# zetareticula/diffusion-llm-rs

Hardware: AMD Instinct MI355X
Metric: int4 dequant+GEMM GiB/s & tok/s per denoise step, 4096×4096, 1/2/4/8 GPU (higher is better)
Workload: dtype f16 X x exact int4 weights (f32 group scales), f32 accumulate; 1 GPU; int4-g128 dequant+GEMM, M=4096 tokens x K=4096 x N=4096; M=4096, K=4096, N=4096, bits=4, group=128, parallelism=column-parallel (hidden dim) x1

## Files before the change

diffusion-llm-rs_amd/csrc/lab/attn_v4.inc:

```

template <int LAB = 0>
__global__ void __launch_bounds__(kWaves * 64)
kv_attention_kernel(const _Float16 *__restrict__ Q, const uint8_t *__restrict__ img, const float *__restrict__ kp,
                    const float *__restrict__ vp, int S, int H, _Float16 *__restrict__ O) {
    const int nkb = (S + kKB - 1) / kKB;
    __shared__ __attribute__((aligned(16))) AttnSmem sm;
    const int tid = threadIdx.x, lane = tid & 63, wave = tid >> 6;
    const int h = blockIdx.y;
    const int q0 = blockIdx.x * kQT + wave * 32;
    const int ql = lane & 31, hh = lane >> 5;
    const float ks = kp[0], vs = vp[0];
    const float c = 1.4426950408889634f * ks / sqrtf(static_cast<float>(kD));

    half8_t qf[kD / 16];
    {
        const int qrow = min(q0 + ql, S - 1);
        const _Float16 *qp = Q + (static_cast<size_t>(qrow) * H + h) * kD + 8 * hh;
#pragma unroll
        for (int t = 0; t < kD / 16; ++t) qf[t] = *reinterpret_cast<const half8_t *>(qp + 16 * t);
    }

    float16_t o[kD / 32];
#pragma unroll
    for (int dt = 0; dt < kD / 32; ++dt)
#pragma unroll
        for (int e = 0; e < 16; ++e) o[dt][e] = 0.0f;
    float m_run = -INFINITY, l_run = 0.0f;

    auto qk = [&](float16_t (&st)[2], const _Float16 (&kb_)[kKB][kKRow]) {
#pragma unroll
        for (int u = 0; u < 2; ++u) {
#pragma unroll
            for (int e = 0; e < 16; ++e) st[u][e] = 0.0f;
#pragma unroll
            for (int t = 0; t < kD / 16; ++t) {
                const half8_t kf = *reinterpret_cast<const half8_t *>(&kb_[32 * u + ql][16 * t + 8 * hh]);
                st[u] = __builtin_amdgcn_mfma_f32_32x32x16_f16(kf, qf[t], st[u], 0, 0, 0);
            }
        }
    };

    const uint8_t *himg = img + static_cast<size_t>(h) * nkb * kImg + lane * 16;
    const uint32_t wv = __builtin_amdgcn_readfirstlane(wave);
    constexpr bool STAG = false;
    auto dma_k = [&](int blk, int buf, uint32_t p0 = 0xffffffffu, uint32_t step = kWaves) {
        const uint8_t *src = himg + static_cast<size_t>(blk) * kImg;
        const uint32_t dst = __builtin_amdgcn_readfirstlane(lds_addr(&sm.k[buf][0][0]));
        for (uint32_t p = p0 == 0xffffffffu ? wv : p0; p < kKImg / 1024; p += step) glds16_asm(src + p * 1024, dst + p * 1024);
    };
    auto dma_v = [&](int blk, int buf, uint32_t p0 = 0xffffffffu, uint32_t step = kWaves) {
        const uint8_t *src = himg + static_cast<size_t>(blk) * kImg + kKImg;
        const uint32_t dst = __builtin_amdgcn_readfirstlane(lds_addr(&sm.vt[buf][0][0]));
        for (uint32_t p = p0 == 0xffffffffu ? wv : p0; p < kVImg / 1024; p += step) glds16_asm(src + p * 1024, dst + p * 1024);
    };
    const bool grp_b = STAG && wave >= kWaves / 2;
    auto raw_barrier = []() __attribute__((always_inline)) {
        asm volatile("s_waitcnt lgkmcnt(0)" ::: "memory");
        __builtin_amdgcn_s_barrier();
        __builtin_amdgcn_sched_barrier(0);
    };
    dma_k(0, 0);
    dma_v(0, 0);
    if (nkb > 1) dma_k(1, 1);
    if (STAG && nkb > 1) dma_v(1, 1);
    asm volatile("s_waitcnt vmcnt(0)" ::: "memory");
    __syncthreads();
    float16_t st[2], sn[2];
    qk(st, sm.k[0]);

    for (int kb = 0; kb < nkb; ++kb) {
        const int j0 = kb * kKB;
        const bool more1 = kb + 1 < nkb, more2 = kb + 2 < nkb;
        if (!(LAB & 2)) {
            if (more2) dma_k(kb + 2, kb & 1);
            if (more1) dma_v(kb + 1, (kb + 1) & 1);
        }
        if (more1) {
            if constexpr (LAB & 8) {
#pragma unroll
                for (int u = 0; u < 2; ++u) sn[u] = st[u] * 0.5f;
            } else {
                qk(sn, sm.k[(kb + 1) & 1]);
            }
        }

        if constexpr (LAB & 1) {
            float lsum = 0.0f;
#pragma unroll
            for (int u = 0; u < 2; ++u)
#pragma unroll
                for (int r = 0; r < 16; ++r) lsum += st[u][r];
            l_run += lsum;
        } else {
        float mloc = -INFINITY;
        if (__builtin_expect(j0 + kKB > S, 0)) {
            asm volatile("" ::: "memory");
#pragma unroll
            for (int u = 0; u < 2; ++u)
#pragma unroll
                for (int r = 0; r < 16; ++r) {
                    const int key = j0 + 32 * u + (r & 3) + 8 * (r >> 2) + 4 * hh;
                    st[u][r] = key < S ? st[u][r] : -INFINITY;
                }
        }
#pragma unroll
        for (int u = 0; u < 2; ++u)
#pragma unroll
            for (int r = 0; r < 16; ++r) mloc = fmaxf(mloc, st[u][r]);
        mloc = fmaxf(mloc, __shfl_xor(mloc, 32, 64));
        const float m_new = fmaxf(m_run, mloc * c);
        const float alpha = __builtin_amdgcn_exp2f(m_run - m_new);
        float lsum = 0.0f;
#pragma unroll
        for (int u = 0; u < 2; ++u)
#pragma unroll
            for (int r = 0; r < 16; ++r) {
                st[u][r] = __builtin_amdgcn_exp2f(fmaf(st[u][r], c, -m_new));
                lsum += st[u][r];
            }
        lsum += __shfl_xor(lsum, 32, 64);
        l_run = l_run * alpha + lsum;
        m_run = m_new;
        if (!__all(alpha == 1.0f)) {
            if (hh == 0) sm.bcast[wave][ql] = alpha;
            __builtin_amdgcn_s_waitcnt(0xC07F);
            __builtin_amdgcn_wave_barrier();
#pragma unroll
            for (int g = 0; g < 4; ++g) {
                const float4 a4 = *reinterpret_cast<const float4 *>(&sm.bcast[wave][8 * g + 4 * hh]);
#pragma unroll
                for (int dt = 0; dt < kD / 32; ++dt) {
                    o[dt][4 * g + 0] *= a4.x; o[dt][4 * g + 1] *= a4.y;
                    o[dt][4 * g + 2] *= a4.z; o[dt][4 * g + 3] *= a4.w;
                }
            }
        }
        }
        const auto &vt = sm.vt[kb & 1];
        if constexpr (!(LAB & 4)) {
// ... 45 lines not shown
```

diffusion-llm-rs_amd/csrc/lab/horner_lab_launch.inc:

```

namespace {

template <int MODE>
void launch_horner_t(const HornerGemmArgs &a, int y_f32, hipStream_t st, int grows = 0) {
    const int nbm = (a.M + 255) / 256, nbn = a.Npad / 256;
    const unsigned nb = static_cast<unsigned>(nbm * nbn);
    const PSampleEpi ep = a.epi ? *a.epi : PSampleEpi{};
    if (a.epi)
        wq_horner_kernel<float, 1, MODE><<<nb, 512, 0, st>>>(a.X, a.M, a.K, a.wdev, a.sz, a.hr, a.sf, a.bias,
                                                             a.epi->x_prev, a.N, a.Npad, nbm, nbn, ep, grows);
    else if (y_f32)
        wq_horner_kernel<float, 0, MODE><<<nb, 512, 0, st>>>(a.X, a.M, a.K, a.wdev, a.sz, a.hr, a.sf, a.bias,
                                                             static_cast<float *>(a.Y), a.N, a.Npad, nbm, nbn, ep,
                                                             grows);
    else
        wq_horner_kernel<__half, 0, MODE><<<nb, 512, 0, st>>>(a.X, a.M, a.K, a.wdev, a.sz, a.hr, a.sf, a.bias,
                                                              static_cast<__half *>(a.Y), a.N, a.Npad, nbm, nbn, ep,
                                                              grows);
}

int launch_horner_lab(const HornerGemmArgs &a, int y_f32, hipStream_t st) {
    if (a.lab == 44 || a.lab == 45) {
        if (a.lab == 44) launch_horner16_t<1 | 256 | 1024 | 2>(a, y_f32, st);
        else launch_horner16_t<1 | 256 | 1024 | 4096>(a, y_f32, st);
        DLLM_LAUNCH_CHECK();
        return DLLM_OK;
    }
    if (a.lab >= 40 && a.lab <= 43) {
        if (a.lab == 40) launch_horner16_t<1 | 256 | 1024 | 4>(a, y_f32, st);
        else if (a.lab == 41) launch_horner16_t<1 | 256 | 1024 | 4 | 8>(a, y_f32, st);
        else if (a.lab == 42) launch_horner16_t<1 | 256 | 1024 | 64>(a, y_f32, st);
        else launch_horner16_t<1 | 256 | 1024 | 2 | 4 | 8 | 64>(a, y_f32, st);
        DLLM_LAUNCH_CHECK();
        return DLLM_OK;
    }
    if (a.lab == 26 || a.lab == 27) {
        if (a.lab == 26) launch_horner16_t<256 | 1024>(a, y_f32, st);
        else launch_horner16_t<1 | 1024>(a, y_f32, st);
        DLLM_LAUNCH_CHECK();
        return DLLM_OK;
    }
    if (a.lab == 25) {
        launch_horner16_t<1 | 256 | 1024 | 2048>(a, y_f32, st);
        DLLM_LAUNCH_CHECK();
        return DLLM_OK;
    }
    if (a.lab == 24) {
        launch_horner16_t<1 | 256>(a, y_f32, st);
        DLLM_LAUNCH_CHECK();
        return DLLM_OK;
    }
    if (a.lab == 21) {
        launch_horner_t<1 | 256>(a, y_f32, st);
        DLLM_LAUNCH_CHECK();
        return DLLM_OK;
    }
    if (a.lab == 19 || a.lab == 20) {
        if (a.lab == 19) launch_horner_t<1 | 256 | 512>(a, y_f32, st);
        else launch_horner_t<3 | 4 | 8 | 16 | 64 | 512>(a, y_f32, st);
        return DLLM_OK;
    }
    if (a.lab == 17 || a.lab == 18) {
        if (a.lab == 17) launch_horner_t<3 | 4 | 8 | 16 | 32>(a, y_f32, st);
        else launch_horner_t<3 | 4 | 8 | 16 | 256>(a, y_f32, st);
        DLLM_LAUNCH_CHECK();
        return DLLM_OK;
    }
    if (a.lab == 16) {
        launch_horner_t<1>(a, y_f32, st);
        DLLM_LAUNCH_CHECK();
        return DLLM_OK;
    }
    if (a.lab == 14 || a.lab == 15) {
        if (a.lab == 14) launch_horner_t<3 | 4 | 8 | 16 | 64>(a, y_f32, st);
        else launch_horner_t<3 | 4 | 8 | 16 | 128>(a, y_f32, st);
        DLLM_LAUNCH_CHECK();
        return DLLM_OK;
    }
    if (a.lab >= 10 && a.lab <= 12) {
        launch_horner_t<1 | 256>(a, y_f32, st, a.lab == 10 ? 4 : a.lab == 11 ? 8 : 16);
        DLLM_LAUNCH_CHECK();
        return DLLM_OK;
    }
    if (a.lab >= 1 && a.lab <= 9) {
        if (a.lab == 1) launch_horner_t<0>(a, y_f32, st);
        else if (a.lab == 2) launch_horner_t<3>(a, y_f32, st);
        else if (a.lab == 3) launch_horner_t<2>(a, y_f32, st);
        else if (a.lab == 4) launch_horner_t<3 | 4>(a, y_f32, st);
        else if (a.lab == 5) launch_horner_t<3 | 8>(a, y_f32, st);
        else if (a.lab == 6) launch_horner_t<3 | 16>(a, y_f32, st);
        else if (a.lab == 7) launch_horner_t<3 | 4 | 8 | 16>(a, y_f32, st);
        else if (a.lab == 8) launch_horner_t<3 | 32>(a, y_f32, st);
        else launch_horner_t<3 | 64>(a, y_f32, st);
        DLLM_LAUNCH_CHECK();
        return DLLM_OK;
    }
    return fail(DLLM_ERR_INVALID_PARAMS, "unknown Horner lab variant");
}

}

int launch_horner_rows_gemm(const HornerGemmArgs &a, int rows, int y_f32, hipStream_t st) {
    if (rows != 128) return fail(DLLM_ERR_INVALID_PARAMS, "Horner tiles: 128 rows");
    launch_horner16_t<1 | 256, 8>(a, y_f32, st);
// ... 5 lines not shown
```

diffusion-llm-rs_amd/csrc/linear_horner.hip:

```cpp
#include "linear_common.hpp"

#include <type_traits>

#ifndef DLLM_LAB
#define DLLM_LAB 0
#endif

namespace dllm {
namespace {

constexpr int kHW = 8 * 1024;
constexpr int kHG = 2048;

__device__ __forceinline__ void horner_burst(__amdgpu_buffer_rsrc_t xr, uint32_t x0, uint32_t x1, uint32_t x2,
                                             uint32_t x3, uint32_t sx, __amdgpu_buffer_rsrc_t wr, uint32_t wo,
                                             uint32_t sw, uint32_t lds0) {
    uint32_t keep;
    asm volatile(
        "s_mov_b32 %0, m0\n\t"
        "s_mov_b32 m0, %9\n\t"
        "s_nop 0\n\t"
        "buffer_load_dwordx4 %1, %5, %6 offen lds\n\t"
        "s_add_u32 m0, m0, 0x2000\n\t"
        "s_nop 0\n\t"
// ... 300 lines not shown
            return;
        }
    }
    if (kg != 0) return;
    const bool vec_ok = (N % 4) == 0;
#pragma unroll
    for (int r = 0; r < 8; ++r) {
        const int m = m0 + r * 32 + (lane & 31);
        if (m >= M) continue;
        YT *yrow = Y + static_cast<size_t>(m) * N;
#pragma unroll
        for (int qd = 0; qd < 4; ++qd)
            store_out4<YT>(yrow, bias, nb0 + 8 * qd, N, vec_ok, acc[r][4 * qd + 0], acc[r][4 * qd + 1],
                           acc[r][4 * qd + 2], acc[r][4 * qd + 3]);
    }
}

typedef float fx4_t __attribute__((ext_vector_type(4)));
typedef uint32_t u32x4_t __attribute__((ext_vector_type(4)));

template <int TB>
__device__ __forceinline__ void store_tile16_f16_lds(uint8_t *img, const fx4_t (&acc)[TB][2], const float4 (&bv)[2],
                                                     __half *Y, int N, int m0, int n0, int wave, int lane) {
    constexpr int kRowB = 512, kCpr = 32;
    const int row16 = lane & 15, rq = lane >> 4;
    constexpr int kTPP = TB < 8 ? TB : 8;
#pragma unroll
    for (int p = 0; p < TB / kTPP; ++p) {
#pragma unroll
        for (int i = 0; i < kTPP; ++i) {
            const int t = 16 * i + row16;
#pragma unroll
            for (int cb = 0; cb < 2; ++cb) {
                const int pc = (4 * wave + 2 * cb + (rq >> 1)) ^ (t & (kCpr - 1));
                const fx4_t &a = acc[kTPP * p + i][cb];
                const float4 &b = bv[cb];
                union { __half h[4]; uint2 u; } pk;
                pk.h[0] = __float2half_rn(a[0] + b.x);
                pk.h[1] = __float2half_rn(a[1] + b.y);
                pk.h[2] = __float2half_rn(a[2] + b.z);
                pk.h[3] = __float2half_rn(a[3] + b.w);
                *reinterpret_cast<uint2 *>(img + t * kRowB + pc * 16 + (rq & 1) * 8) = pk.u;
            }
        }
        __syncthreads();
        const int c = lane % kCpr;
#pragma unroll
        for (int t0 = wave * 2; t0 < 16 * kTPP; t0 += 16) {
            const int t = t0 + lane / kCpr;
            const uint4 v = *reinterpret_cast<const uint4 *>(img + t * kRowB + ((c ^ (t & (kCpr - 1))) * 16));
#if DLLM_NT_STORE
            typedef unsigned int u4nt __attribute__((ext_vector_type(4)));
            __builtin_nontemporal_store(u4nt{v.x, v.y, v.z, v.w},
                                        reinterpret_cast<u4nt *>(Y + static_cast<size_t>(m0 + 16 * kTPP * p + t) * N + n0 + 8 * c));
#else
            *reinterpret_cast<uint4 *>(Y + static_cast<size_t>(m0 + 16 * kTPP * p + t) * N + n0 + 8 * c) = v;
#endif
        }
        __syncthreads();
    }
}

template <int TB>
struct H16 {
    static_assert(TB == 16 || TB == 8, "256- or 128-token tiles");
    static constexpr int kKPS = 16 / TB;
    static constexpr int kXB = 32 * 1024;
    static constexpr int kXSub = kXB / kKPS;
    static constexpr int kWB = kKPS * kHW;
    static constexpr int kStage = kXB + kWB + kHG;
    static constexpr int kNX = TB / 4;
    static constexpr int kPieces = kKPS * (kNX + 1) + 1;
};

template <typename YT, int EPI, int MODE, int TB = 16, int BITS = 4>
__global__ void __launch_bounds__(512, 1)
wq_horner16_kernel(const __half *__restrict__ X, int M, int K, const uint32_t *__restrict__ wdev,
                   const uint32_t *__restrict__ sz, const float *__restrict__ hr, const float *__restrict__ sf,
                   const float *__restrict__ bias, YT *__restrict__ Y, int N, int Npad, int nbm, int nbn,
                   PSampleEpi epi) {
    constexpr bool STAG = MODE & 1;
    static_assert(BITS == 4 || (BITS == 2 && TB == 16), "int4, or int2 on 256-token tiles");
    using L = H16<TB>;
    constexpr int kStage = L::kStage, kXB = L::kXB, kKPS = L::kKPS;
    __shared__ __attribute__((aligned(16))) uint8_t smem[3 * kStage];

    const int nb = nbm * nbn, orig = blockIdx.x;
    const int xcd = orig % kXCDs, q8 = nb / kXCDs, r8 = nb % kXCDs;
    const int tile = (xcd < r8 ? xcd * (q8 + 1) : r8 * (q8 + 1) + (xcd - r8) * q8) + orig / kXCDs;
    const int bm = tile / nbn, bn = tile % nbn;
    const int lane = threadIdx.x & 63;
    const int wave = __builtin_amdgcn_readfirstlane(threadIdx.x >> 6);
    const int m0 = bm * 16 * TB, n0 = bn * 256;
    const int nk = K / kBK;
    const int ns = nk / kKPS;

    uint32_t xo[L::kNX];
#pragma unroll
    for (int i = 0; i < L::kNX; ++i) {
        const int row = (i * 8 + wave) * 8 + (lane >> 3);
        const int rrow = (m0 + row < M ? m0 + row : M - 1) - m0;
        const int c = (lane & 7) ^ ((row >> 1) & 5);
        xo[i] = static_cast<uint32_t>((rrow * K + c * 8) * 2);
    }
    const __amdgpu_buffer_rsrc_t xr = raw_rsrc(X + static_cast<size_t>(m0) * K);
    const uint32_t nt = static_cast<uint32_t>(n0 + 32 * wave) >> 5;
    const __amdgpu_buffer_rsrc_t wr = raw_rsrc(wdev + static_cast<size_t>(nt) * nk * 64 * BITS);
    auto wsoff = [](int kstep) { return static_cast<uint32_t>(BITS == 4 ? kstep * 1024 : (kstep & ~1) * 512); };
    const uint32_t wo = static_cast<uint32_t>(lane * 16);
    const __amdgpu_buffer_rsrc_t gr =
        raw_rsrc(wave == 0 ? static_cast<const void *>(sz + n0) : static_cast<const void *>(hr + n0));
    const bool has_g = wave < 2;
    const uint32_t sbase = __builtin_amdgcn_readfirstlane(lds_addr(smem));

    auto piece = [&](int p, int slot, int st, bool gf) __attribute__((always_inline)) {
        const uint32_t base = sbase + static_cast<uint32_t>(slot * kStage);
        constexpr int nxp = kKPS * L::kNX;
        if (p < nxp) {
            const int kk = p / L::kNX, i = p % L::kNX;
            blds16_asm(xr, xo[i], static_cast<uint32_t>((st * kKPS + kk) * kBK * 2),
                       base + static_cast<uint32_t>(kk * L::kXSub + wave * 1024 + i * 0x2000));
        } else if (p < nxp + kKPS) {
            const int kk = p - nxp;
            blds16_asm(wr, wo, wsoff(st * kKPS + kk),
                       base + static_cast<uint32_t>(kXB + kk * kHW + wave * 1024));
        } else if (p == nxp + kKPS && gf && has_g) {
            blds16_asm(gr, wo, static_cast<uint32_t>(((st * kKPS) >> 1) * Npad * 4),
                       base + static_cast<uint32_t>(kXB + L::kWB + wave * 1024));
        }
    };
    auto stage = [&](int slot, int st, bool gf) __attribute__((always_inline)) {
        if constexpr (TB == 16) {
            horner_burst(xr, xo[0], xo[1], xo[2], xo[3], static_cast<uint32_t>(st * kBK * 2), wr, wo,
                         wsoff(st), sbase + static_cast<uint32_t>(slot * kStage + wave * 1024));
            piece(L::kPieces - 1, slot, st, gf);
        } else {
#pragma unroll
            for (int p = 0; p < L::kPieces; ++p) piece(p, slot, st, gf);
        }
    };

    fx4_t acc[TB][2];
#pragma unroll
    for (int t = 0; t < TB; ++t)
#pragma unroll
        for (int cb = 0; cb < 2; ++cb) acc[t][cb] = fx4_t{0.f, 0.f, 0.f, 0.f};

    const int row16 = lane & 15, rq = lane >> 4;
    const int cq = ((rq & 1) << 1) | (rq >> 1);
    int soff[2];
#pragma unroll
    for (int h = 0; h < 2; ++h) soff[h] = row16 * (kBK * 2) + (((4 * h + cq) ^ ((row16 >> 1) & 5)) << 4);

    auto sj_kk = [](int j) { return TB == 16 ? 0 : (j >> 1); };
    auto sj_h = [](int j) { return TB == 16 ? (j >> 1) : (j & 1); };
    auto sj_tb0 = [](int j) { return TB == 16 ? 8 * (j & 1) : 0; };
    auto read_b = [&](half8_t (&b)[8], const uint8_t *sb, int j) __attribute__((always_inline)) {
#pragma unroll
        for (int i = 0; i < 8; ++i)
            b[i] = *reinterpret_cast<const half8_t *>(sb + sj_kk(j) * L::kXSub + soff[sj_h(j)] +
                                                      (sj_tb0(j) + i) * 16 * kBK * 2);
    };

    ExactConsts ec;
    uint32_t w[BITS];
    float4 r4[2];
    half8_t bA[8], bB[8], a00, a01, a10, a11;
    auto load_w = [&](const uint8_t *sb, int kk, int par) __attribute__((always_inline)) {
        if constexpr (BITS == 4) {
            (void)par;
            const uint4 v = *reinterpret_cast<const uint4 *>(sb + kXB + kk * kHW + wave * 1024 + lane * 16);
            w[0] = v.x; w[1] = v.y; w[2] = v.z; w[3] = v.w;
        } else {
            const uint2 v = *reinterpret_cast<const uint2 *>(sb + kXB + kk * kHW + wave * 1024 + par * 512 + lane * 8);
            w[0] = v.x; w[1] = v.y;
        }
    };
    auto make_a = [&](int h, half8_t &c0, half8_t &c1) __attribute__((always_inline)) {
        u32x4_t u0 = __builtin_bit_cast(u32x4_t, dequant_exact<BITS>(w, 2 * h, ec));
        u32x4_t u1 = __builtin_bit_cast(u32x4_t, dequant_exact<BITS>(w, 2 * h + 1, ec));
#pragma unroll
        for (int e = 0; e < 4; ++e) {
            const auto r = __builtin_amdgcn_permlane16_swap(u0[e], u1[e], false, false);
            u0[e] = r[0];
            u1[e] = r[1];
        }
        c0 = __builtin_bit_cast(half8_t, u0);
        c1 = __builtin_bit_cast(half8_t, u1);
    };
    bool a_done = false;
    int pend_slot = 0, pend_st = 0;
    bool pend_gf = false, pend_on = false;
    constexpr int kPPS = (L::kPieces + 1) / 2;
    auto mma = [&](int t, int cb, const half8_t &a, const half8_t &b) __attribute__((always_inline)) {
        acc[t][cb] = __builtin_amdgcn_mfma_f32_16x16x32_f16(a, b, acc[t][cb], 0, 0, 0);
    };
    auto rescale = [&](int t) __attribute__((always_inline)) {
#pragma unroll
        for (int cb = 0; cb < 2; ++cb) {
            acc[t][cb][0] *= r4[cb].x;
            acc[t][cb][1] *= r4[cb].y;
            acc[t][cb][2] *= r4[cb].z;
            acc[t][cb][3] *= r4[cb].w;
        }
    };
    auto sub = [&](const uint8_t *sb, half8_t (&bc)[8], half8_t (&bn)[8], int j, bool gf) __attribute__((always_inline)) {
        const int tb0 = sj_tb0(j);
        const bool use1 = TB == 16 ? (j >= 2) : (j & 1);
        const half8_t &a0 = use1 ? a10 : a00;
        const half8_t &a1 = use1 ? a11 : a01;
        __builtin_amdgcn_sched_barrier(0);
        if ((MODE & 1024) == 0 && TB == 16 && j == 2 && !((MODE & 8) && a_done)) {
            make_a(1, a10, a11);
            __builtin_amdgcn_sched_barrier(0);
        }
        if (TB == 8 && j == 1) load_w(sb, 1, 1);
        __builtin_amdgcn_s_setprio(1);
        if (TB == 8 && j < 3) {
            if (j & 1) make_a(0, a00, a01);
            else make_a(1, a10, a11);
        }
        if ((MODE & 256) != 0 && j >= 2) {
#pragma unroll
            for (int q = 0; q < 4; ++q) {
                if (j < 3) {
                    const uint8_t *nb = sb + sj_kk(j + 1) * L::kXSub + soff[sj_h(j + 1)] + sj_tb0(j + 1) * 16 * kBK * 2;
                    bn[2 * q] = *reinterpret_cast<const half8_t *>(nb + (2 * q) * 16 * kBK * 2);
                    bn[2 * q + 1] = *reinterpret_cast<const half8_t *>(nb + (2 * q + 1) * 16 * kBK * 2);
                }
                mma(tb0 + 2 * q, 0, a0, bc[2 * q]);
                mma(tb0 + 2 * q, 1, a1, bc[2 * q]);
                mma(tb0 + 2 * q + 1, 0, a0, bc[2 * q + 1]);
                mma(tb0 + 2 * q + 1, 1, a1, bc[2 * q + 1]);
                __builtin_amdgcn_sched_group_barrier(0x008, 2, 0);
                __builtin_amdgcn_sched_group_barrier(0x100, 1, 0);
                __builtin_amdgcn_sched_group_barrier(0x002, 3, 0);
                __builtin_amdgcn_sched_group_barrier(0x008, 2, 0);
                __builtin_amdgcn_sched_group_barrier(0x100, 1, 0);
                __builtin_amdgcn_sched_group_barrier(0x002, 3, 0);
                __builtin_amdgcn_sched_barrier(0);
                if (pend_on && q < kPPS) piece(kPPS * (j - 2) + q, pend_slot, pend_st, pend_gf);
                __builtin_amdgcn_sched_barrier(0);
            }
            __builtin_amdgcn_s_setprio(0);
            __builtin_amdgcn_sched_barrier(0);
            return;
        }
        if (j < 3) read_b(bn, sb, j + 1);
        if (gf && (TB == 16 ? j < 2 : j == 0)) {
#pragma unroll
            for (int i = 0; i < 8; ++i) {
                if constexpr ((MODE & 4) == 0) rescale(tb0 + i);
                mma(tb0 + i, 0, a0, bc[i]);
                mma(tb0 + i, 1, a1, bc[i]);
            }
            __builtin_amdgcn_sched_group_barrier(0x002, 8, 0);
#pragma unroll
            for (int i = 0; i < 8; ++i) {
                if (i + 1 < 8) __builtin_amdgcn_sched_group_barrier(0x002, 8, 0);
                __builtin_amdgcn_sched_group_barrier(0x008, 2, 0);
                __builtin_amdgcn_sched_group_barrier(0x100, 1, 0);
                __builtin_amdgcn_sched_group_barrier(0x002, 1, 0);
            }
        } else {
#pragma unroll
            for (int i = 0; i < 8; ++i) {
                mma(tb0 + i, 0, a0, bc[i]);
                mma(tb0 + i, 1, a1, bc[i]);
            }
#pragma unroll
            for (int i = 0; i < 8; ++i) {
                __builtin_amdgcn_sched_group_barrier(0x008, 2, 0);
                __builtin_amdgcn_sched_group_barrier(0x100, 1, 0);
                __builtin_amdgcn_sched_group_barrier(0x002, 3, 0);
            }
        }
        __builtin_amdgcn_s_setprio(0);
        __builtin_amdgcn_sched_barrier(0);
    };
    auto barrier = []() __attribute__((always_inline)) {
        asm volatile("s_waitcnt lgkmcnt(0)" ::: "memory");
        __builtin_amdgcn_s_barrier();
        __builtin_amdgcn_sched_barrier(0);
    };
    auto wait_one_stage = [&](bool gf) __attribute__((always_inline)) {
        if constexpr (TB == 16) {
            if (gf && has_g) asm volatile("s_waitcnt vmcnt(6)" ::: "memory");
            else asm volatile("s_waitcnt vmcnt(5)" ::: "memory");
        } else {
            if (gf && has_g) asm volatile("s_waitcnt vmcnt(7)" ::: "memory");
            else asm volatile("s_waitcnt vmcnt(6)" ::: "memory");
        }
    };
    const bool grp_b = STAG && wave >= 4;
    auto step = [&](int slot, int si, auto gf_tag) __attribute__((always_inline)) {
        constexpr bool GF = decltype(gf_tag)::value;
        const bool issue = (MODE & 64) == 0 && si + 2 < ns;
        if (!STAG && issue) stage((slot + 2) % 3, si + 2, GF);
        const uint8_t *sb = smem + slot * kStage;
        constexpr bool kEarly = (MODE & 2048) != 0 && TB == 16;
        if (!(kEarly && !GF)) load_w(sb, 0, si & 1);
        if constexpr (GF) {
            half2_t nz, sc;
            split_sz(*reinterpret_cast<const uint32_t *>(sb + kXB + L::kWB + (wave * 32 + (lane & 31)) * 4), nz, sc);
            ec = exact_consts(nz);
            const float *rl = reinterpret_cast<const float *>(sb + kXB + L::kWB + 1024) + wave * 32 + 4 * rq;
            r4[0] = *reinterpret_cast<const float4 *>(rl);
            r4[1] = *reinterpret_cast<const float4 *>(rl + 16);
        }
        read_b(bA, sb, 0);
        if (!(kEarly && !GF) && !((MODE & 8) && a_done)) make_a(0, a00, a01);
        sub(sb, bA, bB, 0, GF);
        sub(sb, bB, bA, 1, GF);
        if constexpr (TB == 16 && (MODE & 1024) != 0) {
            if (!((MODE & 8) && a_done)) make_a(1, a10, a11);
            __builtin_amdgcn_sched_barrier(0);
        }
        if constexpr ((MODE & 8) != 0) a_done = true;
        if constexpr (STAG) {
            if (grp_b) asm volatile("s_waitcnt vmcnt(0)" ::: "memory");
            barrier();
            if constexpr ((MODE & 256) != 0) {
                pend_on = issue;
                pend_slot = (slot + 2) % 3;
                pend_st = si + 2;
                pend_gf = GF;
            } else if (issue) {
                stage((slot + 2) % 3, si + 2, GF);
            }
        }
        sub(sb, bA, bB, 2, GF);
        sub(sb, bB, bA, 3, GF);
        if (!grp_b) {
            if (issue) wait_one_stage(GF);
            else asm volatile("s_waitcnt vmcnt(0)" ::: "memory");
        }
        if constexpr (kEarly && GF) {
            __builtin_amdgcn_sched_barrier(0);
            load_w(smem + ((slot + 1) % 3) * kStage, 0, (si + 1) & 1);
            make_a(0, a00, a01);
            __builtin_amdgcn_sched_barrier(0);
        }
        barrier();
    };

    stage(0, 0, true);
    stage(1, 1, TB == 8);
    wait_one_stage(TB == 8);
    __builtin_amdgcn_s_barrier();
    __builtin_amdgcn_sched_barrier(0);
    if (grp_b) barrier();
    using GFt = std::integral_constant<bool, true>;
    using GFf = std::integral_constant<bool, false>;
    if constexpr (TB == 16) {
        for (int si = 0; si < ns; si += 6) {
            step(0, si, GFt{});
            step(1, si + 1, GFf{});
            if (si + 2 < ns) {
                step(2, si + 2, GFt{});
                step(0, si + 3, GFf{});
            }
            if (si + 4 < ns) {
                step(1, si + 4, GFt{});
                step(2, si + 5, GFf{});
            }
        }
    } else {
        for (int si = 0; si < ns; si += 3) {
            step(0, si, GFt{});
            if (si + 1 < ns) step(1, si + 1, GFt{});
            if (si + 2 < ns) step(2, si + 2, GFt{});
        }
    }
    if (STAG && !grp_b) barrier();

    const int nc0 = n0 + wave * 32 + 4 * rq;
    const float *sl = sf + static_cast<size_t>(nk / 2 - 1) * Npad + nc0;
    float4 bv[2];
#pragma unroll
    for (int cb = 0; cb < 2; ++cb) {
        const float4 s = *reinterpret_cast<const float4 *>(sl + 16 * cb);
        bv[cb] = *reinterpret_cast<const float4 *>(bias + nc0 + 16 * cb);
#pragma unroll
        for (int t = 0; t < TB; ++t) {
            acc[t][cb][0] *= s.x;
            acc[t][cb][1] *= s.y;
            acc[t][cb][2] *= s.z;
            acc[t][cb][3] *= s.w;
        }
    }
    if constexpr ((MODE & 2) != 0) {
#pragma unroll
        for (int t = 0; t < TB; ++t)
#pragma unroll
            for (int cb = 0; cb < 2; ++cb) asm volatile("" ::"v"(acc[t][cb]));
        return;
    }
    if constexpr (EPI == 1) {
#pragma unroll
        for (int t = 0; t < TB; ++t) {
            const int m = m0 + 16 * t + row16;
            if (m >= M) continue;
#pragma unroll
            for (int cb = 0; cb < 2; ++cb) {
                if (nc0 + 16 * cb >= N) continue;
                psample4(epi, m, nc0 + 16 * cb, N, acc[t][cb][0] + bv[cb].x, acc[t][cb][1] + bv[cb].y,
                         acc[t][cb][2] + bv[cb].z, acc[t][cb][3] + bv[cb].w);
            }
        }
        return;
    }
    const bool full = (m0 + 16 * TB <= M) && (n0 + 256 <= N) && (N % 4) == 0;
    if constexpr (std::is_same<YT, __half>::value && (MODE & 4096) == 0) {
        if (full && (N % 8) == 0) {
            store_tile16_f16_lds<TB>(smem, acc, bv, Y, N, m0, n0, wave, lane);
            return;
        }
    }
    if (full) {
#pragma unroll
        for (int t = 0; t < TB; ++t) {
            YT *yrow = Y + static_cast<size_t>(m0 + 16 * t + row16) * N + nc0;
#pragma unroll
            for (int cb = 0; cb < 2; ++cb)
                store4<YT>(yrow + 16 * cb, acc[t][cb][0] + bv[cb].x, acc[t][cb][1] + bv[cb].y,
                           acc[t][cb][2] + bv[cb].z, acc[t][cb][3] + bv[cb].w);
        }
    } else {
        const bool vec_ok = (N % 4) == 0;
#pragma unroll
        for (int t = 0; t < TB; ++t) {
            const int m = m0 + 16 * t + row16;
            if (m >= M) continue;
            YT *yrow = Y + static_cast<size_t>(m) * N;
#pragma unroll
            for (int cb = 0; cb < 2; ++cb)
                store_out4<YT>(yrow, bias, nc0 + 16 * cb, N, vec_ok, acc[t][cb][0], acc[t][cb][1], acc[t][cb][2],
                               acc[t][cb][3]);
        }
    }
}

template <int MODE, int TB = 16, int BITS = 4>
void launch_horner16_t(const HornerGemmArgs &a, int y_f32, hipStream_t st) {
    const int nbm = (a.M + 16 * TB - 1) / (16 * TB), nbn = a.Npad / 256;
    const unsigned nb = static_cast<unsigned>(nbm * nbn);
    const PSampleEpi ep = a.epi ? *a.epi : PSampleEpi{};
    if (a.epi)
        wq_horner16_kernel<float, 1, MODE, TB, BITS><<<nb, 512, 0, st>>>(a.X, a.M, a.K, a.wdev, a.sz, a.hr, a.sf, a.bias,
                                                               a.epi->x_prev, a.N, a.Npad, nbm, nbn, ep);
    else if (y_f32)
        wq_horner16_kernel<float, 0, MODE, TB, BITS><<<nb, 512, 0, st>>>(a.X, a.M, a.K, a.wdev, a.sz, a.hr, a.sf, a.bias,
                                                               static_cast<float *>(a.Y), a.N, a.Npad, nbm, nbn, ep);
    else
        wq_horner16_kernel<__half, 0, MODE, TB, BITS><<<nb, 512, 0, st>>>(a.X, a.M, a.K, a.wdev, a.sz, a.hr, a.sf, a.bias,
                                                                static_cast<__half *>(a.Y), a.N, a.Npad, nbm, nbn, ep);
}

}

int launch_horner_kg2_gemm(const HornerGemmArgs &a, int y_f32, hipStream_t st) {
    const int nbm = (a.M + 255) / 256, nbn = a.Npad / 128;
    const unsigned nb = static_cast<unsigned>(nbm * nbn);
    const PSampleEpi ep = a.epi ? *a.epi : PSampleEpi{};
    if (a.epi)
        wq_horner_kg2_kernel<float, 1><<<nb, 512, 0, st>>>(a.X, a.M, a.K, a.wdev, a.sz, a.hr, a.sf, a.bias,
                                                          a.epi->x_prev, a.N, a.Npad, nbm, nbn, ep);
    else if (y_f32)
        wq_horner_kg2_kernel<float, 0><<<nb, 512, 0, st>>>(a.X, a.M, a.K, a.wdev, a.sz, a.hr, a.sf, a.bias,
                                                          static_cast<float *>(a.Y), a.N, a.Npad, nbm, nbn, ep);
    else
        wq_horner_kg2_kernel<__half, 0><<<nb, 512, 0, st>>>(a.X, a.M, a.K, a.wdev, a.sz, a.hr, a.sf, a.bias,
                                                           static_cast<__half *>(a.Y), a.N, a.Npad, nbm, nbn, ep);
    DLLM_LAUNCH_CHECK();
    return DLLM_OK;
}

#if DLLM_LAB
#include "lab/horner_lab_launch.inc"
#endif

int launch_horner_gemm(const HornerGemmArgs &a, int y_f32, hipStream_t st) {
#if DLLM_LAB
    if (a.lab && a.bits == 4) return launch_horner_lab(a, y_f32, st);
#endif
    if (a.bits == 2) launch_horner16_t<1 | 256 | 1024, 16, 2>(a, y_f32, st);
    else launch_horner16_t<1 | 256 | 1024>(a, y_f32, st);
    DLLM_LAUNCH_CHECK();
    return DLLM_OK;
}

}
```

diffusion-llm-rs_amd/csrc/linear_wq.hip:

```cpp
#include "linear_common.hpp"
#include "stamp.hpp"
#include "diffusion_rng.hpp"
#if DLLM_LAB
#include "dllm_quant_lab.h"
#endif

#ifndef DLLM_LAB
#define DLLM_LAB 0
#endif
#ifndef DLLM_EXACT_HORNER
#define DLLM_EXACT_HORNER 0
#endif
#ifndef DLLM_HORNER_SPLIT
#define DLLM_HORNER_SPLIT 0
#endif
#ifndef DLLM_HORNER_HR_GF
#define DLLM_HORNER_HR_GF 0
#endif
#if DLLM_HORNER_HR_GF && DLLM_HORNER_SPLIT
#error "DLLM_HORNER_SPLIT reads the next group's ratios in every group's second stage"
#endif

#include <algorithm>
#include <atomic>
// ... 1247 lines not shown
#if DLLM_LAB
    if (hc->variant == 14 || hc->variant == 28) return false;
#endif
    const int t128 = ((M + 127) / 128) * (np / 256);
    if (horner_ready(hc, M)) return false;
    if (t128 >= kCUs) return true;
    if (!DLLM_POLICY_ROUNDS || np % 128 != 0 || hc->K % 256 != 0) return false;
    const int tk = ((M + 127) / 128) * (np / 128);
    return 178 * ((t128 + kCUs - 1) / kCUs) <= 100 * ((tk + kCUs - 1) / kCUs);
#else
    (void)hc; (void)M;
    return false;
#endif
}

#ifndef DLLM_HORNER_PC_KG2
#define DLLM_HORNER_PC_KG2 1
#endif
#ifndef DLLM_PC_KG2_MINFILL
#define DLLM_PC_KG2_MINFILL (3 * kCUs / 4)
#endif
#ifndef DLLM_PC_KG2_SMALL
#define DLLM_PC_KG2_SMALL 0
#endif
int horner_pc_kg2_rows(const PlanShape *hc, int M) {
#if DLLM_HORNER_PC_KG2
    const int np = static_cast<int>(hc->Npad);
    if (!(hc->precision == DLLM_PRECISION_EXACT && hc->bits == 4 && hc->group == 128 && hc->K % 256 == 0 &&
          np % 128 == 0 && hc->horner_ok))
        return 0;
#if DLLM_LAB
    if (hc->variant == 14 || hc->variant == 28) return 0;
#endif
    if (horner_ready(hc, M) || horner_pc_ready(hc, M) || horner_kg2_ready(hc, M)) return 0;
#if DLLM_PC_KG2_SMALL
    for (int rows = 128; rows >= 32; rows /= 2) {
        const int t = ((M + rows - 1) / rows) * (np / 128);
        if (t >= 2 * kCUs) return 0;
        if (t >= DLLM_PC_KG2_MINFILL) return rows;
    }
    return 0;
#else
    const int t128 = ((M + 127) / 128) * (np / 128), t64 = ((M + 63) / 64) * (np / 128);
    if (t128 >= 2 * kCUs) return 0;
    if (t128 >= kCUs || t64 > kCUs) return 128;
    return t64 >= DLLM_PC_KG2_MINFILL ? 64 : 0;
#endif
#else
    (void)hc; (void)M;
    return 0;
#endif
}

template <typename YT, int EPI>
int launch_horner(const dllm_linear *h, const __half *X, int M, YT *Y, hipStream_t st, const PSampleEpi *epi) {
#if DLLM_LAB
    const PSampleEpi ep = epi ? *epi : PSampleEpi{};
    if (lab_horner128() && h->bits == 4) {
        const int nbm = (M + 127) / 128, nbn = static_cast<int>(h->Npad / 256);
        wq_gemm8_kernel<4, YT, 8, 4, false, 1, 0, EPI, true><<<static_cast<unsigned>(nbm * nbn), 512, 0, st>>>(
            X, M, (int)h->K, h->wdev, h->sz, h->bias, Y, (int)h->N, (int)h->Npad, (int)h->group, nbm, nbn, 1, nullptr,
            ep, h->hr, h->sf);
        DLLM_LAUNCH_CHECK();
        return DLLM_OK;
    }
    if (h->variant == 24 && h->bits == 4) {
        const int nbm = (M + 255) / 256, nbn = static_cast<int>(h->Npad / 256);
        wq_gemm8_kernel<4, YT, 8, 8, false, 1, 0, EPI, true><<<static_cast<unsigned>(nbm * nbn), 512, 0, st>>>(
            X, M, (int)h->K, h->wdev, h->sz, h->bias, Y, (int)h->N, (int)h->Npad, (int)h->group, nbm, nbn, 1, nullptr,
            ep, h->hr, h->sf);
        DLLM_LAUNCH_CHECK();
        return DLLM_OK;
    }
#endif
    HornerGemmArgs a{X, M, (int)h->K, h->wdev, h->sz, h->hr, h->sf, h->bias, Y, (int)h->N, (int)h->Npad, epi};
    a.bits = static_cast<int>(h->bits);
#if DLLM_LAB
    if (h->variant >= 25 && h->variant <= 27) a.lab = h->variant - 24;
    if (h->variant >= 29 && h->variant <= 31) a.lab = h->variant - 25;
    if (h->variant >= 303 && h->variant <= 304) a.lab = h->variant - 295;
    if (h->variant >= 310 && h->variant <= 312) a.lab = h->variant - 300;
    if ((h->variant >= 314 && h->variant <= 321) || (h->variant >= 324 && h->variant <= 328)) a.lab = h->variant - 300;
    if (h->variant == 305) a.lab = 7;
    if (h->variant >= 340 && h->variant <= 345) a.lab = h->variant - 300;
#endif
    return launch_horner_gemm(a, std::is_same<YT, float>::value ? 1 : 0, st);
}

inline ExactGemmArgs exact_args(const dllm_linear *h, const __half *X, int M, void *Y, const PSampleEpi *epi) {
    ExactGemmArgs a{h->bits, X, M, (int)h->K, h->wdev, h->sz, h->sf, h->bias, Y, (int)h->N, (int)h->Npad,
                    (int)h->group, epi};
#if DLLM_LAB
    a.tm = h->variant == 15 ? 1 : 0;
    a.lab_policy = h->variant == 28 ? 1 : (h->variant >= 300 && h->variant <= 302 ? h->variant - 298 : (h->variant == 329 ? 5 : (h->variant == 330 ? 6 : (h->variant == 331 ? 7 : 0))));
#endif
    return a;
}

inline void prefill_plan(const PlanShape *h, int M, dllm_linear_plan_t *p) {
    if (!use_exact(h)) return rounded_plan(h, M, p);
    auto horner = [&](int kernel, int tm, int tn, int kg) {
        p->kernel = kernel;
        p->tile_m = tm; p->tile_n = tn; p->kgroups = kg; p->nsplit = 1;
        p->flags = 0;
    };
    if ((h->bits == 4 || h->bits == 2) && horner_ready(h, M)) return horner(DLLM_KERNEL_HORNER16, 256, 256, 1);
    if (h->bits == 4 && horner_pc_ready(h, M)) return horner(DLLM_KERNEL_HORNER_PC, 128, 256, 1);
    if (h->bits == 4 && horner_kg2_ready(h, M)) return horner(DLLM_KERNEL_HORNER_KG2, 256, 128, 2);
    if (const int rows = h->bits == 4 ? horner_pc_kg2_rows(h, M) : 0)
        return horner(DLLM_KERNEL_HORNER_PC_KG2, rows, 128, 2);
    select_exact_plan(h->bits, M, static_cast<int>(h->K), static_cast<int>(h->Npad), static_cast<int>(h->group), p);
}

inline void select_plan(const PlanShape *h, size_t M, int fused, dllm_linear_plan_t *p) {
    if (M <= static_cast<size_t>(kDecodeMaxM) && h->decode_layout) decode_plan(h, static_cast<int>(M), p);
    else prefill_plan(h, static_cast<int>(M), p);
    if (fused && M <= static_cast<size_t>(kDecodeMaxM)) p->flags |= DLLM_PLAN_NOT_FUSED;
}

template <int BITS, typename YT, int EPI = 0>
int launch_prefill_auto(const dllm_linear *h, const __half *X, int M, YT *Y, hipStream_t st,
                        const dllm_linear_plan_t &p, const PSampleEpi *epi = nullptr) {
#if DLLM_LAB
    if (h->variant == 4) {
        const PlanShape s = plan_shape_of(h);
        dllm_linear_plan_t rp;
        rounded_plan(&s, M, &rp);
        return launch_rounded<BITS, YT, EPI>(h, X, M, Y, st, rp, epi);
    }
    if ((h->variant == 14 || h->variant == 15) && exact_gemm_supported(M, (int)h->K, (int)h->Npad, (int)h->group))
        return launch_exact_gemm(exact_args(h, X, M, Y, epi), std::is_same<YT, float>::value ? 1 : 0, st);
    if (h->variant >= 0) {
        const int rc = launch_lab_variant<BITS, YT, EPI>(h, X, M, Y, st, epi);
        if (rc >= 0) return rc;
    }
#endif
    const int y_f32 = std::is_same<YT, float>::value ? 1 : 0;
    const HornerGemmArgs ha{X, M, (int)h->K, h->wdev, h->sz, h->hr, h->sf, h->bias, Y, (int)h->N, (int)h->Npad, epi};
    switch (p.kernel) {
    case DLLM_KERNEL_HORNER16:
        if constexpr (BITS == 4 || BITS == 2) return launch_horner<YT, EPI>(h, X, M, Y, st, epi);
        break;
    case DLLM_KERNEL_HORNER_PC:
        if constexpr (BITS == 4) return launch_horner_pc_gemm(ha, y_f32, st);
        break;
    case DLLM_KERNEL_HORNER_KG2:
        if constexpr (BITS == 4) return launch_horner_kg2_gemm(ha, y_f32, st);
        break;
    case DLLM_KERNEL_HORNER_PC_KG2:
        if constexpr (BITS == 4) return launch_horner_pc_kg2_gemm(ha, p.tile_m, y_f32, st);
        break;
    case DLLM_KERNEL_EXACT_FOLD: {
#if DLLM_LAB
        const PlanShape s = plan_shape_of(h);
        if (const int rows = BITS == 4 ? horner_rows(&s, M) : 0)
            return launch_horner_rows_gemm(ha, rows, y_f32, st);
#endif
        ExactGemmArgs a = exact_args(h, X, M, Y, epi);
#if DLLM_EXACT_HORNER
        if (BITS == 4 && h->hstate == 1) a.hr = h->hr;
#endif
        return launch_exact_gemm(a, y_f32, st);
    }
    case DLLM_KERNEL_ROUNDED_RING: return launch_rounded<BITS, YT, EPI>(h, X, M, Y, st, p, epi);
    default: break;
    }
    return fail(DLLM_ERR_UNSUPPORTED, "linear forward: no kernel for the plan");
// ... 345 lines not shown
        DLLM_LAUNCH_CHECK();
    }
    return DLLM_OK;
}

int dllm_linear_info(dllm_linear_t h, size_t *K, size_t *N, uint8_t *bits, size_t *group) {
    if (!h) return fail(DLLM_ERR_INVALID_PARAMS, "null handle");
    if (K) *K = h->K;
    if (N) *N = h->N;
    if (bits) *bits = static_cast<uint8_t>(h->bits);
    if (group) *group = h->group;
    return DLLM_OK;
}

int dllm_linear_plan(dllm_linear_t h, size_t M, int fused, dllm_linear_plan_t *out) {
    if (!h || !out) return fail(DLLM_ERR_INVALID_PARAMS, "null argument");
    if (M == 0 || M > (1u << 30)) return fail(DLLM_ERR_SHAPE_MISMATCH, "M must be 1..2^30");
    if (fused && h->N % 4) return fail(DLLM_ERR_UNSUPPORTED, "fused p_sample needs N % 4 == 0");
    const PlanShape s = plan_shape_of(h);
    select_plan(&s, M, fused, out);
    return DLLM_OK;
}

int dllm_linear_plan_shape(size_t K, size_t N, uint8_t bits, size_t group, int flags, int horner_ok, size_t M,
                           int fused, dllm_linear_plan_t *out) {
    if (!out) return fail(DLLM_ERR_INVALID_PARAMS, "null argument");
    if (const int rc = check_shape(K, N, bits, group, flags)) return rc;
    if (M == 0 || M > (1u << 30)) return fail(DLLM_ERR_SHAPE_MISMATCH, "M must be 1..2^30");
    if (fused && N % 4) return fail(DLLM_ERR_UNSUPPORTED, "fused p_sample needs N % 4 == 0");
    PlanShape s;
    s.K = K; s.N = N; s.Npad = (N + kBN - 1) / kBN * kBN; s.group = group;
    s.bits = bits; s.precision = flags & ~DLLM_LINEAR_PREFILL_ONLY;
    s.decode_layout = (flags & DLLM_LINEAR_PREFILL_ONLY) == 0;
    s.horner_ok = horner_ok != 0 && horner_shape(&s);
    select_plan(&s, M, fused, out);
    return DLLM_OK;
}

int dllm_linear_precision(dllm_linear_t h) {
    if (!h) {
        fail(DLLM_ERR_INVALID_PARAMS, "null handle");
        return -1;
    }
    return h->precision;
}

size_t dllm_linear_weight_bytes(dllm_linear_t h) {
    if (!h) return 0;
    return h->Npad * h->K * h->bits / 8 + h->G * h->Npad * (use_exact(h) ? 8 : 4);
}

size_t dllm_linear_device_bytes(dllm_linear_t h) {
    if (!h) return 0;
    size_t b = h->Npad * h->K * h->bits / 8 + h->G * h->Npad * 8 + h->Npad * 4;
    if (h->wdec) b += h->Npad * ((h->K + 127) / 128) * 128 * h->bits / 8;
    if (h->hr) b += (h->G + 1) * h->Npad * 4;
#if DLLM_LAB
    b += h->Npad * h->K * h->bits / 8;
#endif
    return b;
}

#if DLLM_LAB
int dllm_linear_set_kernel_variant(dllm_linear_t h, int variant) {
    if (!h) return fail(DLLM_ERR_INVALID_PARAMS, "null handle");
    if (variant >= 200 && variant < 264) {
        h->dcfg = variant - 199;
        return DLLM_OK;
    }
    if (variant >= 16 && variant < 24) {
        h->dlab = variant - 16;
        return DLLM_OK;
    }
    if (variant >= 32 && variant < 96) {
        h->rlab = variant - 32;
        return DLLM_OK;
    }
    if (variant >= 100 && variant < 196) {
        h->variant = 9 + (variant - 100) / 32;
        h->pplab = (variant - 100) % 32;
        return DLLM_OK;
    }
    if (variant < -1 || (variant > 15 && (variant < 24 || variant > 31) && (variant < 300 || variant > 331 || variant == 313) &&
                         (variant < 340 || variant > 345)))
        return fail(DLLM_ERR_INVALID_PARAMS, "variant must be -1..15, 24..31, 300..312, 314..331 or 340..345 (16..23, 32..95, 100..195, 200..263: ablations)");
    h->variant = variant;
    h->dlab = h->rlab = h->pplab = h->dcfg = 0;
    return DLLM_OK;
}
#endif

int dllm_linear_destroy(dllm_linear_t h) {
    free_linear(h);
    return DLLM_OK;
}

}
```

Measured before the change: 38.63 million tok/s.

## Add four-slot LDS ring pipeline to horner16 int4 GEMM and make it default

```diff
diff --git a/diffusion-llm-rs_amd/csrc/lab/attn_v4.inc b/diffusion-llm-rs_amd/csrc/lab/attn_v4.inc
--- a/diffusion-llm-rs_amd/csrc/lab/attn_v4.inc
+++ b/diffusion-llm-rs_amd/csrc/lab/attn_v4.inc
@@ -53,8 +53,8 @@
         const uint32_t dst = __builtin_amdgcn_readfirstlane(lds_addr(&sm.vt[buf][0][0]));
         for (uint32_t p = p0 == 0xffffffffu ? wv : p0; p < kVImg / 1024; p += step) glds16_asm(src + p * 1024, dst + p * 1024);
     };
-    const bool grp_b = STAG && wave >= kWaves / 2;
-    auto raw_barrier = []() __attribute__((always_inline)) {
+    [[maybe_unused]] const bool grp_b = STAG && wave >= kWaves / 2;
+    [[maybe_unused]] auto raw_barrier = []() __attribute__((always_inline)) {
         asm volatile("s_waitcnt lgkmcnt(0)" ::: "memory");
         __builtin_amdgcn_s_barrier();
         __builtin_amdgcn_sched_barrier(0);
diff --git a/diffusion-llm-rs_amd/csrc/lab/horner_lab_launch.inc b/diffusion-llm-rs_amd/csrc/lab/horner_lab_launch.inc
--- a/diffusion-llm-rs_amd/csrc/lab/horner_lab_launch.inc
+++ b/diffusion-llm-rs_amd/csrc/lab/horner_lab_launch.inc
@@ -20,6 +20,13 @@
 }
 
 int launch_horner_lab(const HornerGemmArgs &a, int y_f32, hipStream_t st) {
+    if (a.lab >= 46 && a.lab <= 48) {
+        if (a.lab == 46) launch_horner16_t<kH16Ring4>(a, y_f32, st);
+        else if (a.lab == 47) launch_horner16_t<kH16Ring4Skew>(a, y_f32, st);
+        else launch_horner16_t<kH16Ring3>(a, y_f32, st);
+        DLLM_LAUNCH_CHECK();
+        return DLLM_OK;
+    }
     if (a.lab == 44 || a.lab == 45) {
         if (a.lab == 44) launch_horner16_t<1 | 256 | 1024 | 2>(a, y_f32, st);
         else launch_horner16_t<1 | 256 | 1024 | 4096>(a, y_f32, st);
diff --git a/diffusion-llm-rs_amd/csrc/linear_horner.hip b/diffusion-llm-rs_amd/csrc/linear_horner.hip
--- a/diffusion-llm-rs_amd/csrc/linear_horner.hip
+++ b/diffusion-llm-rs_amd/csrc/linear_horner.hip
@@ -406,8 +406,14 @@
     constexpr bool STAG = MODE & 1;
     static_assert(BITS == 4 || (BITS == 2 && TB == 16), "int4, or int2 on 256-token tiles");
     using L = H16<TB>;
-    constexpr int kStage = L::kStage, kXB = L::kXB, kKPS = L::kKPS;
-    __shared__ __attribute__((aligned(16))) uint8_t smem[3 * kStage];
+    constexpr bool RING4 = (MODE & 8192) != 0;
+    static_assert(!RING4 || (TB == 16 && (MODE & (256 | 1024)) == (256 | 1024) && (MODE & (2048 | 64 | 8)) == 0),
+                  "the 4-slot ring: 256-token tiles, spread pieces, half 1's A fragments after substep 1");
+    constexpr int kXB = L::kXB, kKPS = L::kKPS;
+    constexpr int kStage = RING4 ? kXB + kHG : L::kStage;
+    constexpr int kGOff = RING4 ? kXB : kXB + L::kWB;
+    constexpr int kWRing = 4 * (kXB + kHG);
+    __shared__ __attribute__((aligned(16))) uint8_t smem[RING4 ? kWRing + 8 * 3 * 1024 : 3 * kStage];
 
     const int nb = nbm * nbn, orig = blockIdx.x;
     const int xcd = orig % kXCDs, q8 = nb / kXCDs, r8 = nb % kXCDs;
@@ -436,11 +442,22 @@
         raw_rsrc(wave == 0 ? static_cast<const void *>(sz + n0) : static_cast<const void *>(hr + n0));
     const bool has_g = wave < 2;
     const uint32_t sbase = __builtin_amdgcn_readfirstlane(lds_addr(smem));
+    const __amdgpu_buffer_rsrc_t gr4 = raw_rsrc(wave < 4 ? static_cast<const void *>(sz + n0 + 64 * wave)
+                                                         : static_cast<const void *>(hr + n0 + 64 * (wave - 4)));
+    uint32_t wq = 0, wq_iss = 2048;
 
     auto piece = [&](int p, int slot, int st, bool gf) __attribute__((always_inline)) {
         const uint32_t base = sbase + static_cast<uint32_t>(slot * kStage);
         constexpr int nxp = kKPS * L::kNX;
-        if (p < nxp) {
+        if constexpr (RING4) {
+            if (p < 4)
+                blds16_asm(xr, xo[p], static_cast<uint32_t>(st * kBK * 2), base + static_cast<uint32_t>(wave * 1024 + p * 0x2000));
+            else if (p == 4)
+                blds16_asm(wr, wo, wsoff(st), sbase + static_cast<uint32_t>(kWRing + wave * 3072) + wq_iss);
+            else if (p == 5 && gf)
+                blds4_asm(gr4, static_cast<uint32_t>(lane * 4), static_cast<uint32_t>((st >> 1) * Npad * 4),
+                          base + static_cast<uint32_t>(kXB + wave * 256));
+        } else if (p < nxp) {
             const int kk = p / L::kNX, i = p % L::kNX;
             blds16_asm(xr, xo[i], static_cast<uint32_t>((st * kKPS + kk) * kBK * 2),
                        base + static_cast<uint32_t>(kk * L::kXSub + wave * 1024 + i * 0x2000));
@@ -491,7 +508,16 @@
     float4 r4[2];
     half8_t bA[8], bB[8], a00, a01, a10, a11;
     auto load_w = [&](const uint8_t *sb, int kk, int par) __attribute__((always_inline)) {
-        if constexpr (BITS == 4) {
+        if constexpr (RING4) {
+            const uint8_t *wp = smem + kWRing + wave * 3072 + wq;
+            if constexpr (BITS == 4) {
+                const uint4 v = *reinterpret_cast<const uint4 *>(wp + lane * 16);
+                w[0] = v.x; w[1] = v.y; w[2] = v.z; w[3] = v.w;
+            } else {
+                const uint2 v = *reinterpret_cast<const uint2 *>(wp + par * 512 + lane * 8);
+                w[0] = v.x; w[1] = v.y;
+            }
+        } else if constexpr (BITS == 4) {
             (void)par;
             const uint4 v = *reinterpret_cast<const uint4 *>(sb + kXB + kk * kHW + wave * 1024 + lane * 16);
             w[0] = v.x; w[1] = v.y; w[2] = v.z; w[3] = v.w;
@@ -626,9 +652,9 @@
         if (!(kEarly && !GF)) load_w(sb, 0, si & 1);
         if constexpr (GF) {
             half2_t nz, sc;
-            split_sz(*reinterpret_cast<const uint32_t *>(sb + kXB + L::kWB + (wave * 32 + (lane & 31)) * 4), nz, sc);
+            split_sz(*reinterpret_cast<const uint32_t *>(sb + kGOff + (wave * 32 + (lane & 31)) * 4), nz, sc);
             ec = exact_consts(nz);
-            const float *rl = reinterpret_cast<const float *>(sb + kXB + L::kWB + 1024) + wave * 32 + 4 * rq;
+            const float *rl = reinterpret_cast<const float *>(sb + kGOff + 1024) + wave * 32 + 4 * rq;
             r4[0] = *reinterpret_cast<const float4 *>(rl);
             r4[1] = *reinterpret_cast<const float4 *>(rl + 16);
         }
@@ -668,35 +694,107 @@
         barrier();
     };
 
-    stage(0, 0, true);
-    stage(1, 1, TB == 8);
-    wait_one_stage(TB == 8);
-    __builtin_amdgcn_s_barrier();
-    __builtin_amdgcn_sched_barrier(0);
-    if (grp_b) barrier();
     using GFt = std::integral_constant<bool, true>;
     using GFf = std::integral_constant<bool, false>;
-    if constexpr (TB == 16) {
-        for (int si = 0; si < ns; si += 6) {
-            step(0, si, GFt{});
-            step(1, si + 1, GFf{});
-            if (si + 2 < ns) {
-                step(2, si + 2, GFt{});
-                step(0, si + 3, GFf{});
-            }
-            if (si + 4 < ns) {
-                step(1, si + 4, GFt{});
-                step(2, si + 5, GFf{});
-            }
-        }
+    if constexpr (RING4) {
+        auto h1 = [&](int slot, auto gf_tag) __attribute__((always_inline)) {
+            constexpr bool GF = decltype(gf_tag)::value;
+            const uint8_t *sb = smem + slot * kStage;
+            load_w(sb, 0, GF ? 0 : 1);
+            if constexpr (GF) {
+                half2_t nz, sc;
+                split_sz(*reinterpret_cast<const uint32_t *>(sb + kGOff + (wave * 32 + (lane & 31)) * 4), nz, sc);
+                ec = exact_consts(nz);
+                const float *rl = reinterpret_cast<const float *>(sb + kGOff + 1024) + wave * 32 + 4 * rq;
+                r4[0] = *reinterpret_cast<const float4 *>(rl);
+                r4[1] = *reinterpret_cast<const float4 *>(rl + 16);
+            }
+            read_b(bA, sb, 0);
+            make_a(0, a00, a01);
+            sub(sb, bA, bB, 0, GF);
+            sub(sb, bB, bA, 1, GF);
+            make_a(1, a10, a11);
+            __builtin_amdgcn_sched_barrier(0);
+        };
+        auto h2 = [&](int slot, bool issue, int islot, int ist, bool igf) __attribute__((always_inline)) {
+            const uint8_t *sb = smem + slot * kStage;
+            pend_on = issue;
+            pend_slot = islot;
+            pend_st = ist;
+            pend_gf = igf;
+            sub(sb, bA, bB, 2, false);
+            sub(sb, bB, bA, 3, false);
+        };
+        auto interval = [&](auto gf_tag, int kt, auto issue_tag, auto wait_tag) __attribute__((always_inline)) {
+            constexpr bool GF = decltype(gf_tag)::value, ISSUE = decltype(issue_tag)::value,
+                           WAIT = decltype(wait_tag)::value;
+            const int slot = kt & 3, islot = (kt + 2) & 3;
+            if (grp_b && (!GF || kt > 0)) h2((kt + 3) & 3, ISSUE, islot, kt + 2, GF);
+            h1(slot, gf_tag);
+            if (!WAIT || !grp_b) h2(slot, ISSUE, islot, kt + 2, GF);
+            if constexpr (WAIT) {
+                if constexpr (!ISSUE) asm volatile("s_waitcnt vmcnt(0)" ::: "memory");
+                else if constexpr (GF) asm volatile("s_waitcnt vmcnt(6)" ::: "memory");
+                else asm volatile("s_waitcnt vmcnt(5)" ::: "memory");
+                __builtin_amdgcn_s_barrier();
+                __builtin_amdgcn_sched_barrier(0);
+            }
+            wq = wq == 2048 ? 0 : wq + 1024;
+            wq_iss = wq_iss == 2048 ? 0 : wq_iss + 1024;
+        };
+        wq_iss = 0;
+#pragma unroll
+        for (int p = 0; p < L::kPieces; ++p) piece(p, 0, 0, true);
+        wq_iss = 1024;
+#pragma unroll
+        for (int p = 0; p < L::kPieces; ++p) piece(p, 1, 1, false);
+        wq_iss = 2048;
+        const int ni = ns - 2;
+        if (grp_b && ni > 0) {
+#pragma unroll
+            for (int p = 0; p < L::kPieces; ++p) piece(p, 2, 2, true);
+            asm volatile("s_waitcnt vmcnt(11)" ::: "memory");
+        } else {
+            asm volatile("s_waitcnt vmcnt(5)" ::: "memory");
+        }
+        __builtin_amdgcn_s_barrier();
+        __builtin_amdgcn_sched_barrier(0);
+        for (int kt = 0; kt < ni; kt += 2) {
+            interval(GFt{}, kt, GFt{}, GFt{});
+            interval(GFf{}, kt + 1, GFt{}, GFt{});
+        }
+        interval(GFt{}, ni, GFf{}, GFt{});
+        interval(GFf{}, ni + 1, GFf{}, GFf{});
+        barrier();
     } else {
-        for (int si = 0; si < ns; si += 3) {
-            step(0, si, GFt{});
-            if (si + 1 < ns) step(1, si + 1, GFt{});
-            if (si + 2 < ns) step(2, si + 2, GFt{});
-        }
-    }
-    if (STAG && !grp_b) barrier();
+        stage(0, 0, true);
+        stage(1, 1, TB == 8);
+        wait_one_stage(TB == 8);
+        __builtin_amdgcn_s_barrier();
+        __builtin_amdgcn_sched_barrier(0);
+        if (grp_b) barrier();
+        if constexpr (TB == 16) {
+            for (int si = 0; si < ns; si += 6) {
+                step(0, si, GFt{});
+                step(1, si + 1, GFf{});
+                if (si + 2 < ns) {
+                    step(2, si + 2, GFt{});
+                    step(0, si + 3, GFf{});
+                }
+                if (si + 4 < ns) {
+                    step(1, si + 4, GFt{});
+                    step(2, si + 5, GFf{});
+                }
+            }
+        } else {
+            for (int si = 0; si < ns; si += 3) {
+                step(0, si, GFt{});
+                if (si + 1 < ns) step(1, si + 1, GFt{});
+                if (si + 2 < ns) step(2, si + 2, GFt{});
+            }
+        }
+        if (STAG && !grp_b) barrier();
+    }
 
     const int nc0 = n0 + wave * 32 + 4 * rq;
     const float *sl = sf + static_cast<size_t>(nk / 2 - 1) * Npad + nc0;
@@ -764,6 +862,11 @@
         }
     }
 }
+
+[[maybe_unused]] constexpr int kH16Ring3 = 1 | 256 | 1024;
+[[maybe_unused]] constexpr int kH16Ring4 = 256 | 1024 | 8192;
+[[maybe_unused]] constexpr int kH16Ring4Skew = 1 | 256 | 1024 | 8192;
+constexpr int kH16Arm = kH16Ring4Skew;
 
 template <int MODE, int TB = 16, int BITS = 4>
 void launch_horner16_t(const HornerGemmArgs &a, int y_f32, hipStream_t st) {
@@ -808,8 +911,8 @@
 #if DLLM_LAB
     if (a.lab && a.bits == 4) return launch_horner_lab(a, y_f32, st);
 #endif
-    if (a.bits == 2) launch_horner16_t<1 | 256 | 1024, 16, 2>(a, y_f32, st);
-    else launch_horner16_t<1 | 256 | 1024>(a, y_f32, st);
+    if (a.bits == 2) launch_horner16_t<kH16Arm, 16, 2>(a, y_f32, st);
+    else launch_horner16_t<kH16Arm>(a, y_f32, st);
     DLLM_LAUNCH_CHECK();
     return DLLM_OK;
 }
diff --git a/diffusion-llm-rs_amd/csrc/linear_wq.hip b/diffusion-llm-rs_amd/csrc/linear_wq.hip
--- a/diffusion-llm-rs_amd/csrc/linear_wq.hip
+++ b/diffusion-llm-rs_amd/csrc/linear_wq.hip
@@ -1353,7 +1353,7 @@
     if (h->variant >= 310 && h->variant <= 312) a.lab = h->variant - 300;
     if ((h->variant >= 314 && h->variant <= 321) || (h->variant >= 324 && h->variant <= 328)) a.lab = h->variant - 300;
     if (h->variant == 305) a.lab = 7;
-    if (h->variant >= 340 && h->variant <= 345) a.lab = h->variant - 300;
+    if (h->variant >= 340 && h->variant <= 348) a.lab = h->variant - 300;
 #endif
     return launch_horner_gemm(a, std::is_same<YT, float>::value ? 1 : 0, st);
 }
@@ -1865,8 +1865,8 @@
         return DLLM_OK;
     }
     if (variant < -1 || (variant > 15 && (variant < 24 || variant > 31) && (variant < 300 || variant > 331 || variant == 313) &&
-                         (variant < 340 || variant > 345)))
-        return fail(DLLM_ERR_INVALID_PARAMS, "variant must be -1..15, 24..31, 300..312, 314..331 or 340..345 (16..23, 32..95, 100..195, 200..263: ablations)");
+                         (variant < 340 || variant > 348)))
+        return fail(DLLM_ERR_INVALID_PARAMS, "variant must be -1..15, 24..31, 300..312, 314..331 or 340..348 (16..23, 32..95, 100..195, 200..263: ablations)");
     h->variant = variant;
     h->dlab = h->rlab = h->pplab = h->dcfg = 0;
     return DLLM_OK;
```

Result: faster. 39.71 million tok/s (median of 6 runs) (+2.8%).
